# frankenz/Deep-convolutional-neural-network-ResNet-26-and-Attention-network

Measured on AMD Instinct MI355X. Metric: tiles/sec fwd+bwd, 256x256x3 bags, ResNet-26+attn, higher is better.
Workload: dtype bf16; 1 GPU; 8 bags x 256 tiles @256x256x3 per GPU, ResNet-26 (20/40/60/80) + attention-MIL head, fwd+bwd full-bag path (BASELINE.json configs[1]); global_bags=8, tiles_per_bag=256, tile=256, parallelism=bag-parallel dp1, one RCCL all-reduce of the flat 2.56 MB gradient bucket

## Files before the change

### deep-convolutional-neural-network-resnet-26-and-attention-network_amd/_lib.py

```python
import contextlib
import ctypes
import os
import subprocess
import threading

import torch

_HERE = os.path.dirname(os.path.abspath(__file__))
LIB_PATH = os.environ.get("MIL_LIB_PATH") or os.path.join(_HERE, "libmil_hip.so")
POISON_LIB_PATH = os.path.join(_HERE, "libmil_hip_poison.so")

MIL_DT_F32, MIL_DT_BF16, MIL_DT_BF16_DGRAD, MIL_DT_F32S, MIL_DT_F32S_DGRAD = 0, 1, 2, 3, 4
BF16X3 = "bf16x3"
PACK_FWD, PACK_DGRAD, PACK_STEM, PACK_DGRAD_S2 = 0, 1, 2, 3
_ERR = {1: "invalid argument", 2: "unsupported shape / channel configuration", 3: "kernel launch failed"}


class MilLibraryError(RuntimeError):
    pass


def build_library(verbose=False, poison=False):
    cmd = ["make", "-C", os.path.join(_HERE, "csrc"), "-j", str(min(8, os.cpu_count() or 1))] + (["POISON=1"] if poison else [])
    res = subprocess.run(cmd, stdout=subprocess.PIPE, stderr=subprocess.STDOUT, text=True)
    out = POISON_LIB_PATH if poison else os.path.join(_HERE, "libmil_hip.so")
    if verbose or res.returncode != 0:
        print(res.stdout)
    if res.returncode != 0:
        raise MilLibraryError(f"building {os.path.basename(out)} failed")
    return out


_c = ctypes
_vp, _i, _f, _sz = _c.c_void_p, _c.c_int, _c.c_float, _c.c_size_t
_SIGS = {
    "mil_abi_version": ([], _i),
    "mil_stream_copy": ([_vp, _vp, _sz, _vp], _i),
    "mil_split_probe": ([_vp, _vp, _vp, _i, _vp], _i),
    "mil_stem_s2d": ([_vp, _vp, _i, _i, _i, _i, _vp], _i),
    "mil_u8_decode_table": ([_vp], _i),
    "mil_stem_s2d_u8": ([_vp, _vp, _i, _i, _i, _i, _vp], _i),
    "mil_packed_weight_elems": ([_c.POINTER(_sz), _i, _i, _i, _i], _i),
    "mil_pack_conv_weights": ([_vp, _vp, _vp, _vp, _i, _i, _i, _i, _i, _vp], _i),
    "mil_conv_igemm": ([_vp] * 6 + [_i] * 12 + [_f, _i, _vp], _i),
    "mil_conv_wgrad_workspace": ([_c.POINTER(_sz)] + [_i] * 12, _i),
    "mil_conv_wgrad": ([_vp, _vp, _vp, _vp, _vp, _sz] + [_i] * 13 + [_vp], _i),
    "mil_reduce_job_bytes": ([], _i),
    "mil_reduce_defer_begin": ([_vp, _i], _i),
    "mil_reduce_defer_end": ([_c.POINTER(_i)], _i),
    "mil_wgrad_reduce_all": ([_vp, _vp, _i, _vp], _i),
    "mil_conv_bwd_fused_workspace": ([_c.POINTER(_sz)] + [_i] * 8, _i),
    "mil_conv_bwd_fused": ([_vp] * 8 + [_sz] + [_i] * 9 + [_f, _i, _vp], _i),
    "mil_maxpool_fwd": ([_vp, _vp, _vp, _i, _i, _i, _i, _i, _vp], _i),
    "mil_maxpool_bwd": ([_vp, _vp, _vp, _i, _i, _i, _i, _i, _f, _i, _vp], _i),
    "mil_resize_plan": ([_i, _i, _c.POINTER(_i)], _i),
    "mil_resize_coeffs": ([_i, _i, _vp, _vp], _i),
    "mil_tile_preprocess": ([_vp, _vp, _vp, _vp, _vp, _vp, _i, _i, _i, _i, _vp], _i),
    "mil_tile_preprocess_s2d": ([_vp, _vp, _vp, _vp, _vp, _vp, _i, _i, _i, _i, _vp], _i),
    "mil_tile_preprocess_u8": ([_vp, _vp, _vp, _vp, _vp, _vp, _i, _i, _i, _i, _vp], _i),
    "mil_tile_preprocess_win": ([_vp, _c.c_int64, _vp, _c.c_int64, _vp, _vp, _vp, _vp, _vp, _i, _i, _i, _i, _vp], _i),
    "mil_tile_preprocess_win_s2d": ([_vp, _c.c_int64, _vp, _c.c_int64, _vp, _vp, _vp, _vp, _vp, _i, _i, _i, _i, _vp], _i),
    "mil_tile_preprocess_win_u8": ([_vp, _c.c_int64, _vp, _c.c_int64, _vp, _vp, _vp, _vp, _vp, _i, _i, _i, _i, _vp], _i),
    "mil_roi_stats": ([_vp, _c.c_int64, _vp, _c.c_int64, _i, _i, _i, _i, _i, _vp, _vp], _i),
    "mil_stem_fwd_fused_xs": ([_vp, _vp, _vp, _vp, _vp, _i, _i, _i, _i, _f, _i, _vp], _i),
    "mil_stem_fwd_fused_u8": ([_vp, _vp, _vp, _vp, _vp, _i, _i, _i, _i, _f, _i, _vp], _i),
    "mil_conv_block_fwd": ([_vp, _vp, _vp, _vp, _vp, _vp, _vp, _i, _i, _i, _i, _f, _i, _vp], _i),
    "mil_conv_chain": ([_vp, _vp, _i, _i, _i, _i, _i, _f, _i, _vp], _i),
    "mil_conv_pair": ([_vp, _vp, _vp, _vp, _vp, _i, _vp, _vp, _vp, _vp, _vp, _i, _vp, _i, _i, _i, _i, _f, _i, _vp], _i),
    "mil_conv_s2_entry": ([_vp, _vp, _vp, _vp, _vp, _vp, _i, _i, _i, _i, _i, _f, _i, _vp], _i),
    "mil_conv_wgrad_pair_workspace": ([_c.POINTER(_sz), _i, _i, _i, _i, _i, _i, _i, _i], _i),
    "mil_conv_wgrad_pair": ([_vp, _vp, _vp, _vp, _vp, _vp, _vp, _sz, _i, _i, _i, _i, _i, _i, _i, _i, _i, _vp], _i),
    "mil_conv_dgrad_s2": ([_vp, _vp, _vp, _vp, _vp, _i, _i, _i, _i, _i, _i, _i, _f, _i, _vp], _i),
    "mil_stem_fwd_fused": ([_vp, _vp, _vp, _vp, _vp, _vp, _i, _i, _i, _i, _f, _i, _vp], _i),
    "mil_stem_bwd_fused_workspace": ([_c.POINTER(_sz), _i, _i, _i, _i], _i),
    "mil_stem_bwd_fused": ([_vp, _vp, _vp, _vp, _vp, _vp, _sz, _i, _i, _i, _f, _i, _i, _vp], _i),
    "mil_stem_bwd_fused_nchw_workspace": ([_c.POINTER(_sz), _i, _i, _i, _i], _i),
    "mil_stem_bwd_fused_nchw": ([_vp, _vp, _vp, _vp, _vp, _vp, _sz, _i, _i, _i, _f, _i, _i, _vp], _i),
    "mil_stem_bwd_fused_u8_workspace": ([_c.POINTER(_sz), _i, _i, _i, _i], _i),
    "mil_stem_bwd_fused_u8": ([_vp, _vp, _vp, _vp, _vp, _vp, _sz, _i, _i, _i, _f, _i, _i, _vp], _i),
# ... 99 lines not shown
```

### deep-convolutional-neural-network-resnet-26-and-attention-network_amd/csrc/conv_wgrad.hip

```cpp
#include "pf_common.cuh"
#include "reduce.cuh"
#include "stamp.cuh"
#include "u8_feed.cuh"

template <typename T>
struct WgradArgs {
    const typename T::elem* x;
    const typename T::elem* dz;
    float* slab;
    ConvGeom g;
    int ntiles;
    int tile_px;
    int lds_z_off;
    unsigned x_bytes, z_bytes;
    const typename T::elem* dz2;
    int lds_z2_off;
    unsigned long long* stamp;
};

__device__ __forceinline__ bf16x8_t tr_pair(const char* p0, const char* p1) {
    typedef __attribute__((address_space(3))) s16x4_t lds_s16x4;
    s16x4_t lo = __builtin_amdgcn_ds_read_tr16_b64_v4i16((lds_s16x4*)(p0));
    s16x4_t hi = __builtin_amdgcn_ds_read_tr16_b64_v4i16((lds_s16x4*)(p1));
    typedef __attribute__((ext_vector_type(8))) short s16x8_t;
    s16x8_t v = __builtin_shufflevector(lo, hi, 0, 1, 2, 3, 4, 5, 6, 7);
    return __builtin_bit_cast(bf16x8_t, v);
}

__host__ __device__ constexpr bool mil_wgrad_x3_half(bool split, int ks, int cinp, int nt, int msplit, bool proj) {
    return split && ks == 3 && cinp == 40 && nt == 3 && msplit == 1 && !proj;
}
__host__ __device__ constexpr int mil_wgrad_halo_max(int cinp, bool proj, bool split = false, bool half = false) {
    if ((split && cinp >= 64) || half) return 200;
    return (proj && cinp <= 24) ? 576 : 400;
}
__host__ __device__ constexpr int mil_wgrad_tile_max(int cinp, bool split, bool half = false) { return ((split && cinp >= 64) || half) ? 128 : 256; }
constexpr int MIL_WGRAD_X3_WAVES = 2;
template <typename T, int KS, int CINP, int NT, int MSPLIT, bool PF, int NW = 4, bool PROJ = false>
__global__ __launch_bounds__(64 * NW, NW == 8 ? ((T::SPLIT && CINP <= 24 && NT <= 2) ? MIL_WGRAD_X3_WAVES : 2) : ((PF && CINP > 40) ? 1 : ((PF && T::SPLIT) ? 2 : 0))) void wgrad_kernel(WgradArgs<T> a) {
    extern __shared__ __attribute__((aligned(16))) char smem[];
    MIL_POISON(smem);
    constexpr int ESZ = T::ESZ;
    constexpr int PIXB = mil_pix_pitch(CINP, ESZ);
    constexpr int COUTP = mil_nt_to_cp(NT);
    constexpr int PIXZ = mil_pix_pitch(COUTP, ESZ);
    constexpr int CG = CINP / 8;
    constexpr int RG = KS * KS * CG;
    constexpr int MT = (RG + 1) / 2;
    constexpr int MT_S = (MT + MSPLIT - 1) / MSPLIT;
    constexpr int NTHR = 64 * NW;
    constexpr int MW = (MT_S + NW - 1) / NW;
    constexpr int PM0 = 2 * CG, PM1 = (5 * CG - 1) / 2, PMN = PROJ ? PM1 - PM0 + 1 : 0;
    constexpr bool WPIPE = T::DT == MIL_DT_BF16 && PF && CINP < 64;
    constexpr bool ZFOLD = T::SPLIT && (COUTP % 16) == 8;
    constexpr int ZFOLD_D = COUTP * 2 - 16;
    const ConvGeom& g = a.g;
    const int tid = threadIdx.x, lane = tid & 63;
    const int wave = __builtin_amdgcn_readfirstlane(tid >> 6);
    const int split = blockIdx.y;
    const bool bias_wave = (wave == 0 && split == 0);
    char* ldsX = smem;
    char* ldsZ = smem + a.lds_z_off;

    int toff[MW];
    bool mvalid[MW];
    int proj_i = -1, proj_mt = 0;
#pragma unroll
    for (int i = 0; i < MW; ++i) {
        const int ml = wave + NW * i;
        const int mt = split * MT_S + ml;
        mvalid[i] = (ml < MT_S) && (mt < MT);
        if (PROJ && mvalid[i] && mt >= PM0 && mt <= PM1) { proj_i = i; proj_mt = mt; }
// ... 244 lines not shown
        if (ZFOLD && nt == NT - 1) {
            const float up = __shfl_down(v, 8, 16);
            return col < 8 ? v + up : 0.f;
        }
        return v;
    };
    if constexpr (PROJ) {
        if (proj_i >= 0) {
#pragma unroll
            for (int nt = 0; nt < NT; ++nt)
#pragma unroll
                for (int e = 0; e < 4; ++e)
                    slab[(size_t)((MT + 1 + proj_mt - PM0) * 16 + gq * 4 + e) * SLAB_COLS + nt * 16 + col] = unfold(accp[nt][e], nt);
        }
    }
#pragma unroll
    for (int i = 0; i < MW; ++i) {
        if (!mvalid[i]) continue;
        const int mt = split * MT_S + wave + NW * i;
#pragma unroll
        for (int nt = 0; nt < NT; ++nt)
#pragma unroll
            for (int e = 0; e < 4; ++e)
                slab[(size_t)(mt * 16 + gq * 4 + e) * SLAB_COLS + nt * 16 + col] = unfold(acc[i][nt][e], nt);
    }
    if (bias_wave) {
#pragma unroll
        for (int nt = 0; nt < NT; ++nt)
#pragma unroll
            for (int e = 0; e < 4; ++e)
                slab[(size_t)(MT * 16 + gq * 4 + e) * SLAB_COLS + nt * 16 + col] = unfold(accb[nt][e], nt);
    }
}

static thread_local MilDeferState g_defer{nullptr, 0, 0};
MilDeferState& mil_defer_state() { return g_defer; }

__global__ __launch_bounds__(32 * MIL_RED_GROUPS) void wgrad_reduce_job_kernel(MilReduceJob j) {
    __shared__ f32x4_t part[MIL_RED_GROUPS][32];
    MIL_POISON_STATIC(part);
    mil_reduce_job_block(j, blockIdx.x, part);
}

__global__ __launch_bounds__(32 * MIL_RED_GROUPS) void wgrad_reduce_all_kernel(const MilReduceJob* __restrict__ jobs, int njobs) {
    __shared__ f32x4_t part[MIL_RED_GROUPS][32];
    __shared__ int which;
    MIL_POISON_STATIC(part); MIL_POISON_STATIC(which);
    const int b = blockIdx.x;
    if (threadIdx.x < 64) {
        bool mine = false;
        if ((int)threadIdx.x < njobs) {
            const int b0 = jobs[threadIdx.x].block0, nb = jobs[threadIdx.x].n_blocks;
            mine = b >= b0 && b < b0 + nb;
        }
        const unsigned long long m = __ballot(mine);
        if (threadIdx.x == 0) which = m ? __ffsll((long long)m) - 1 : -1;
    }
    __syncthreads();
    const int k = which;
    if (k < 0) return;
    const MilReduceJob j = jobs[k];
    mil_reduce_job_block(j, b - j.block0, part);
}

extern "C" int mil_reduce_job_bytes(void) { return (int)sizeof(MilReduceJob); }

// ... 184 lines not shown
    if (g.ks == 4 && cinp == 16 && coutp == 24) MIL_WG(4, 16, 2, 1);
    if (g.ks == 4 && cinp == 16 && coutp == 64) MIL_WG(4, 16, 4, 1);
    if (g.ks == 3) {
        if (cinp == 24 && coutp == 24) MIL_WG(3, 24, 2, 1);
        if (cinp == 40 && coutp == 40) MIL_WG(3, 40, 3, 1);
        if (cinp == 64 && coutp == 64) MIL_WG(3, 64, 4, 1);
        if (cinp == 80 && coutp == 80) { if constexpr (T::SPLIT) { MIL_WG(3, 80, 5, 3); } else { MIL_WG(3, 80, 5, 2); } }
        if (cinp == 24 && coutp == 40) MIL_WG(3, 24, 3, 1);
        if (cinp == 40 && coutp == 64) {
            if constexpr (T::SPLIT) { MIL_WG(3, 40, 4, 2); } else { MIL_WG(3, 40, 4, 1); }
        }
        if (cinp == 64 && coutp == 80) MIL_WG(3, 64, 5, 2);
    }
    if (g.ks == 1) {
        if (cinp == 24 && coutp == 40) MIL_WG(1, 24, 3, 1);
        if (cinp == 40 && coutp == 64) MIL_WG(1, 40, 4, 1);
        if (cinp == 64 && coutp == 80) MIL_WG(1, 64, 5, 1);
    }
#undef MIL_WG
    return MIL_ERR_UNSUPPORTED;
}

static int wgrad_entry(const void* x, const void* dz, float* dw, float* db, void* ws, size_t ws_bytes, int n_img,
                       int H, int W, int cin, int Ho, int Wo, int cout, int ks, int stride, int pad, int stem_mode,
                       int accumulate, int dtype, bool query, size_t* need, void* stream) {
    if (n_img < 0 || H <= 0 || W <= 0 || Ho <= 0 || Wo <= 0) return MIL_ERR_ARG;
    ConvGeom g{};
    g.n_img = n_img; g.H = H; g.W = W; g.Ho = Ho; g.Wo = Wo; g.ks = ks; g.stride = stride; g.pad = pad; g.zins = 0;
    hipStream_t st = reinterpret_cast<hipStream_t>(stream);
    if (dtype == MIL_DT_BF16) return dispatch_wgrad<BF16>(x, dz, dw, db, ws, ws_bytes, g, cout, cin, stem_mode, accumulate, query, need, st);
    if (dtype == MIL_DT_F32) return dispatch_wgrad<F32>(x, dz, dw, db, ws, ws_bytes, g, cout, cin, stem_mode, accumulate, query, need, st);
    if (dtype == MIL_DT_F32S) return dispatch_wgrad<F32S>(x, dz, dw, db, ws, ws_bytes, g, cout, cin, stem_mode, accumulate, query, need, st);
    return MIL_ERR_ARG;
}

struct StemBwdArgs {
    const __bf16* xs;
    const float* x;
    const uint8_t* x8;
    int H, W;
    unsigned x_bytes;
    int lds_dump_off;
    const __bf16* gp;
    int gpx;
    const uint8_t* widx;
    float* slab;
    ConvGeom g;
    int Hp, Wp;
    int ntiles;
    int lds_z_off, lds_g_off, lds_i_off;
    unsigned xs_bytes, gp_bytes, wi_bytes;
    float slope;
    unsigned long long* stamp;
};

constexpr int MIL_STEM_BWD_WAVES = 2;
template <bool FROM_X, bool X3, int NPW, bool U8>
__device__ __forceinline__ void stem_bwd_fused_body(const StemBwdArgs& a) {
    extern __shared__ __attribute__((aligned(16))) char smem[];
    MIL_POISON(smem);
    static_assert(!X3 || FROM_X, "the split-precision form reads the fp32 tiles");
    static_assert(!U8 || FROM_X, "the uint8 feed rebuilds its s2d tiles");
    constexpr int CINP = 16, NT = 2, KS = 4, COUTP = 24;
    constexpr int PIXB = mil_pix_pitch(CINP, X3 ? 4 : 2);
    constexpr int PIXZ = mil_pix_pitch(COUTP, X3 ? 4 : 2);
    constexpr int PIXG = 96;
// ... 484 lines not shown
                                     reinterpret_cast<hipStream_t>(stream));
}

extern "C" int mil_conv_wgrad_pair_workspace(size_t* bytes, int n_img, int H, int W, int cin, int Ho, int Wo, int cout, int dtype) {
    if (!bytes) return MIL_ERR_ARG;
    return wgrad_pair_entry(nullptr, nullptr, nullptr, nullptr, nullptr, nullptr, nullptr, 0, n_img, H, W, cin, Ho, Wo, cout, 0,
                            dtype, true, bytes, nullptr);
}

extern "C" int mil_conv_wgrad_pair(const void* x, const void* dz1, const void* dz2, float* dw3, float* db3, float* dw1,
                                   void* workspace, size_t workspace_bytes, int n_img, int H, int W, int cin, int Ho, int Wo,
                                   int cout, int accumulate, int dtype, void* stream) {
    if (!x || !dz1 || !dz2 || !dw3 || !dw1 || !workspace) return MIL_ERR_ARG;
    size_t need = 0;
    return wgrad_pair_entry(x, dz1, dz2, dw3, db3, dw1, workspace, workspace_bytes, n_img, H, W, cin, Ho, Wo, cout, accumulate,
                            dtype, false, &need, stream);
}

extern "C" int mil_conv_wgrad_workspace(size_t* bytes, int n_img, int H, int W, int cin, int Ho, int Wo, int cout,
                                        int ks, int stride, int pad, int stem_mode, int dtype) {
    if (!bytes) return MIL_ERR_ARG;
    return wgrad_entry(nullptr, nullptr, nullptr, nullptr, nullptr, 0, n_img, H, W, cin, Ho, Wo, cout, ks, stride, pad,
                       stem_mode, 0, dtype, true, bytes, nullptr);
}

extern "C" int mil_conv_wgrad(const void* x, const void* dz, float* dw, float* db, void* workspace,
                              size_t workspace_bytes, int n_img, int H, int W, int cin, int Ho, int Wo, int cout,
                              int ks, int stride, int pad, int stem_mode, int accumulate, int dtype, void* stream) {
    if (!x || !dz || !dw) return MIL_ERR_ARG;
    size_t need = 0;
    return wgrad_entry(x, dz, dw, db, workspace, workspace_bytes, n_img, H, W, cin, Ho, Wo, cout, ks, stride, pad,
                       stem_mode, accumulate, dtype, false, &need, stream);
}
```

### deep-convolutional-neural-network-resnet-26-and-attention-network_amd/encoder.py

```python
import contextlib
import os

import torch
from torch import nn

from . import _lib as L
from . import hooks
from . import ops

STAGE_WIDTHS = (20, 40, 60, 80)
WEIGHT_EPOCH = [0]
STEM_WIDTH = 20


def invalidate_packed_weights():
    WEIGHT_EPOCH[0] += 1


class BasicResBlock(nn.Module):
    expansion = 1

    def __init__(self, inplanes, planes, stride=1, downsample=None, groups=1, base_width=64):
        super().__init__()
        if groups != 1 or base_width != 64:
# ... 5 lines not shown
        self.stride = stride

    def forward(self, x):
        raise RuntimeError("BasicResBlock is executed by the fused HIP encoder (ResNet.forward); "
                           "it has no stand-alone torch path")


class ResNet(nn.Module):

    def __init__(self, block=BasicResBlock, layers=(3, 3, 3, 3), num_classes=80, zero_init_residual=False,
                 groups=1, width_per_group=64, compute_dtype=L.BF16X3):
        super().__init__()
        if block is not BasicResBlock or groups != 1 or width_per_group != 64:
            raise ValueError("the HIP encoder implements BasicResBlock with groups=1, base_width=64")
        self.inplanes = STEM_WIDTH
        self.conv1 = nn.Conv2d(3, STEM_WIDTH, kernel_size=7, stride=2, padding=3)
        self.relu = nn.LeakyReLU(ops.LEAK, inplace=True)
        self.maxpool = nn.MaxPool2d(kernel_size=3, stride=2, padding=1)
        for i, (width, depth) in enumerate(zip(STAGE_WIDTHS, layers)):
            setattr(self, f"layer{i + 1}", self._make_layer(width, depth, stride=1 if i == 0 else 2))
        self.avgpool = nn.AdaptiveAvgPool2d((1, 1))
        self.fc = nn.Linear(STAGE_WIDTHS[-1], num_classes, bias=False)
        self.compute_dtype = compute_dtype
        self.overlap_wgrad = False
        self.direct_grad = False
        self.n_side_streams = 1
        self.fuse_backward = True
        self.fuse_stem_forward = True
        self.keep_s2d = False
        self.fuse_stage_entry = True
        self.fuse_block_forward = True
        self.dense_grads = True
        self.batch_reductions = True
        self._reduce_batch = None
        self._pack_table = None
        self._pack_version = None
        self._side = None

    def _make_layer(self, planes, blocks, stride=1):
        shortcut = None
        if stride != 1 or self.inplanes != planes:
            shortcut = nn.Sequential(nn.Conv2d(self.inplanes, planes, kernel_size=1, stride=stride, bias=False))
        seq = [BasicResBlock(self.inplanes, planes, stride, shortcut)]
        self.inplanes = planes
        seq += [BasicResBlock(planes, planes) for _ in range(1, blocks)]
        return nn.Sequential(*seq)

    def blocks(self):
        for i in range(4):
            for blk in getattr(self, f"layer{i + 1}"):
                yield blk

    def encoder_params(self):
        ps = [self.conv1.weight, self.conv1.bias]
        for blk in self.blocks():
            ps += [blk.conv1.weight, blk.conv1.bias, blk.conv2.weight, blk.conv2.bias]
            if blk.downsample is not None:
                ps.append(blk.downsample[0].weight)
        ps.append(self.fc.weight)
        return ps

    def _side_streams(self):
        if self._side is None:
            self._side = [torch.cuda.Stream() for _ in range(self.n_side_streams)]
        return self._side

# ... 261 lines not shown
    batch = None
    if net.batch_reductions and not use_side:
        if net._reduce_batch is None or net._reduce_batch.device != dfeats.device:
            net._reduce_batch = ops.ReduceBatch(dfeats.device)
        batch = net._reduce_batch

    def gout(*params):
        return tuple(None if p is None else p.grad for p in params) if direct else None

    def wgrad(xin, dzz, cin, cout, key=None, **kw):
        n, h, w, _ = xin.shape
        _, ho, wo, _ = dzz.shape
        need = ops.wgrad_workspace_bytes(n, h, w, cin, ho, wo, cout, kw["ks"], kw["stride"], kw["pad"],
                                         kw.get("stem", False), xin.dtype)
        if batch is not None:
            assert key is not None, "deferred reductions need one workspace per call site: pass key="
            return ops.conv_wgrad(xin, dzz, cin, cout, workspace=batch.workspace(("w", key), need), **kw)
        if not use_side:
            if ws[-1] is None or ws[-1].numel() * 4 < need:
                ws[-1] = torch.empty((need + 3) // 4, dtype=torch.float32, device=xin.device)
            return ops.conv_wgrad(xin, dzz, cin, cout, workspace=ws[-1], **kw)
        k = rr[0] % len(sides)
        rr[0] += 1
        side = sides[k]
        side.wait_stream(main)
        with torch.cuda.stream(side):
            if ws[k] is None or ws[k].numel() * 4 < need:
                ws[k] = torch.empty((need + 3) // 4, dtype=torch.float32, device=xin.device)
            out = ops.conv_wgrad(xin, dzz, cin, cout, workspace=ws[k], **kw)
        xin.record_stream(side)
        dzz.record_stream(side)
        return out

    fws = None

    def is_dense(t, c):
        return t.shape[-1] == c and ops.cpad(c) != c

    def fused_bwd(dzz, wd, xin, cin, cout, addend, mask, out, key=None):
        nonlocal fws
        n, h, w, _ = dzz.shape
        dense = is_dense(dzz, cout)
        need = ops.bwd_fused_workspace_bytes(n, h, w, cout, cin, 3, 1, dzz.dtype, dense)
        if need is None:
            if dense:
                raise RuntimeError("dense gradient layout chosen for a shape without a fused backward kernel")
            return None
        if batch is not None:
            return ops.conv_bwd_fused(dzz, wd, xin, cin, cout, addend=addend, mask=mask, workspace=batch.workspace(("f", key), need), out=out)
        if fws is None or fws.numel() * 4 < need:
            fws = torch.empty((need + 3) // 4, dtype=torch.float32, device=dzz.device)
        return ops.conv_bwd_fused(dzz, wd, xin, cin, cout, addend=addend, mask=mask, workspace=fws, out=out)

    def stage_dgrad_chain(bi, dz_out):
        li, j, depth = net.block_position(bi)
        e = bi - depth + 1
        split_ = dtype == torch.float32 and L.dt_code(dtype, mma=True) == L.MIL_DT_F32S
        if j != depth - 1 or depth < 2 or depth > 3 or not net.fuse_backward or not (dtype == torch.bfloat16 or split_):
            return None
        ent = blocks[e]
        if ent.stride != 2 or ent.downsample is None or any(b.stride != 1 or b.downsample is not None for b in blocks[e + 1:bi + 1]):
            return None
        cout = ent.conv1.out_channels
        n, h, w, cp = dz_out.shape
        if (cp, h, w) not in ops.RESIDENT_SHAPES or ops.bwd_fused_workspace_bytes(n, h, w, cout, cout, 3, 1, dtype) is not None:
            return None
        convs, src = [], None
        for k in range(bi, e, -1):
            xin_k, o1_k, _ = saved["blocks"][k]
            w2d_k, _ = net._packed(f"b{k}.c2", blocks[k].conv2.weight, None, L.PACK_DGRAD, dtype)
            w1d_k, _ = net._packed(f"b{k}.c1", blocks[k].conv1.weight, None, L.PACK_DGRAD, dtype)
            convs.append(dict(w=w2d_k, act=o1_k))
            convs.append(dict(w=w1d_k, res=dz_out if src is None else src, act=xin_k))
            src = len(convs) - 1
        _xin_e, o1_e, _ = saved["blocks"][e]
        w2d_e, _ = net._packed(f"b{e}.c2", ent.conv2.weight, None, L.PACK_DGRAD, dtype)
        convs.append(dict(w=w2d_e, act=o1_e))
        outs = ops.conv_chain(dz_out, convs)
        if outs is None:
            return None
        done = {}
        dz_k = dz_out
        for i, k in enumerate(range(bi, e, -1)):
            xin_k, o1_k, _ = saved["blocks"][k]
            dmid_k, dz_prev = outs[2 * i], outs[2 * i + 1]
            grads[f"b{k}.c2"] = wgrad(o1_k, dz_k, cout, cout, key=(k, 2), ks=3, stride=1, pad=1, out=gout(blocks[k].conv2.weight, blocks[k].conv2.bias))
            grads[f"b{k}.c1"] = wgrad(xin_k, dmid_k, cout, cout, key=(k, 1), ks=3, stride=1, pad=1, out=gout(blocks[k].conv1.weight, blocks[k].conv1.bias))
            done[k] = "done"
            dz_k = dz_prev
        grads[f"b{e}.c2"] = wgrad(o1_e, dz_k, cout, cout, key=(e, 2), ks=3, stride=1, pad=1, out=gout(ent.conv2.weight, ent.conv2.bias))
        done[e] = (dz_k, outs[-1])
        return done

    pre = {}
    with (batch if batch is not None else contextlib.nullcontext()):
        for bi in range(len(blocks) - 1, -1, -1):
            blk = blocks[bi]
            xin, o1, _out = saved["blocks"][bi]
            cin, cout, s = blk.conv1.in_channels, blk.conv1.out_channels, blk.stride
            if bi not in pre:
                chain = stage_dgrad_chain(bi, dz)
                if chain is not None:
                    pre.update(chain)
            if pre.get(bi) == "done":
                continue
            w2d, _ = net._packed(f"b{bi}.c2", blk.conv2.weight, None, L.PACK_DGRAD, dtype)
            if bi in pre:
                dz, dz1 = pre[bi]
                fused = "chain"
            else:
                fused = fused_bwd(dz, w2d, o1, cout, cout, None, True, gout(blk.conv2.weight, blk.conv2.bias), key=(bi, 2)) if net.fuse_backward else None
            if fused == "chain":
                pass
            elif fused is not None:
                dz1, grads[f"b{bi}.c2"] = fused[0], (fused[1], fused[2])
            elif is_dense(dz, cout):
                raise RuntimeError("dense gradient layout without the fused backward")
            else:
                grads[f"b{bi}.c2"] = wgrad(o1, dz, cout, cout, key=(bi, 2), ks=3, stride=1, pad=1, out=gout(blk.conv2.weight, blk.conv2.bias))
                if s == 1 and blk.downsample is None and net.fuse_backward:
                    w1d_, _ = net._packed(f"b{bi}.c1", blk.conv1.weight, None, L.PACK_DGRAD, dtype)
                    chain = ops.conv_pair(dz, w2d, None, w1d_, None, actA=o1, resB=dz, actB=xin if bi > 0 else None)
                    if chain is not None:
# ... 106 lines not shown
```

### deep-convolutional-neural-network-resnet-26-and-attention-network_amd/ops.py

```python
import ctypes

import torch

from . import _lib as L

LEAK = 0.1


class KernelTimer:

    def __init__(self, want):
        self.want = want
        self.spans = []

    def bracket(self, label):
        if not self.want(label):
            return None
        start = torch.cuda.Event(enable_timing=True)
        end = torch.cuda.Event(enable_timing=True)
        start.record()
        self.spans.append((label, start, end))
        return end

    def durations_ms(self):
# ... 129 lines not shown


def wgrad_workspace_bytes(n, h, w, cin, ho, wo, cout, ks, stride, pad, stem, dtype):
    need = ctypes.c_size_t(0)
    L.check(L.lib().mil_conv_wgrad_workspace(ctypes.byref(need), n, h, w, cin, ho, wo, cout, ks, stride, pad,
                                             1 if stem else 0, L.dt_code(dtype, mma=True)), "mil_conv_wgrad_workspace")
    return need.value


def conv_wgrad(x, dz, cin, cout, *, ks, stride, pad, stem=False, want_bias=True, workspace=None, out=None):
    n, h, w, cin_p = x.shape
    _, ho, wo, cout_p = dz.shape
    _need(dz, (n, ho, wo, cpad(cout)), x.dtype, "dz")
    _need(x, (n, h, w, 16 if stem else cpad(cin)), x.dtype, "x")
    need = wgrad_workspace_bytes(n, h, w, cin, ho, wo, cout, ks, stride, pad, stem, x.dtype)
    if workspace is None or workspace.numel() * workspace.element_size() < need:
        workspace = torch.empty((need + 3) // 4, dtype=torch.float32, device=x.device)
    kk = 7 if stem else ks
    if out is None:
        dw = torch.empty((cout, cin, kk, kk), dtype=torch.float32, device=x.device)
        db = torch.empty(cout, dtype=torch.float32, device=x.device) if want_bias else None
    else:
        dw, db = out
        _need(dw, (cout, cin, kk, kk), torch.float32, "dw")
        _need(db, (cout,), torch.float32, "db")
    end = TIMER.bracket(("wgrad", cin_p, cout_p, ks, stride, n, ho, wo)) if TIMER else None
    L.check(L.lib().mil_conv_wgrad(x.data_ptr(), dz.data_ptr(), dw.data_ptr(), L.ptr(db), workspace.data_ptr(),
                                   workspace.numel() * workspace.element_size(), n, h, w, cin, ho, wo, cout, ks, stride,
                                   pad, 1 if stem else 0, 0 if out is None else 1, L.dt_code(x.dtype, mma=True), L.stream_ptr()),
            "mil_conv_wgrad")
    if end is not None:
        end.record()
    return dw, db


def bwd_fused_workspace_bytes(n, h, w, cout, cin, ks, pad, dtype, dense=False):
    need = ctypes.c_size_t(0)
    rc = L.lib().mil_conv_bwd_fused_workspace(ctypes.byref(need), n, h, w, cout, cin, ks, pad, L.dt_code(dtype, dense, mma=True))
    if rc == 2:
        return None
    L.check(rc, "mil_conv_bwd_fused_workspace")
    return need.value


def conv_bwd_fused(dz, wpack_dgrad, x, cin, cout, *, addend=None, mask=True, ks=3, pad=1, workspace=None, slope=LEAK,
                   out=None):
    n, h, w, cz = dz.shape
    dense = cz == cout and cpad(cout) != cout
    need = bwd_fused_workspace_bytes(n, h, w, cout, cin, ks, pad, dz.dtype, dense)
    if need is None:
        return None
    _need(dz, (n, h, w, cout if dense else cpad(cout)), dz.dtype, "dz")
    _need(x, (n, h, w, cpad(cin)), dz.dtype, "x")
    _need(addend, (n, h, w, cin if dense else cpad(cin)), dz.dtype, "addend")
    if workspace is None or workspace.numel() * workspace.element_size() < need:
        workspace = torch.empty((need + 3) // 4, dtype=torch.float32, device=dz.device)
    dx = torch.empty((n, h, w, cin), dtype=dz.dtype, device=dz.device) if dense else torch.empty_like(x)
    if out is None:
        dw = torch.empty((cout, cin, ks, ks), dtype=torch.float32, device=dz.device)
        db = torch.empty(cout, dtype=torch.float32, device=dz.device)
    else:
        dw, db = out
        _need(dw, (cout, cin, ks, ks), torch.float32, "dw")
        _need(db, (cout,), torch.float32, "db")
    end = TIMER.bracket(("bwd_fused", cpad(cout), cpad(cin), ks, 1, False, n, h, w, addend is not None)) if TIMER else None
    L.check(L.lib().mil_conv_bwd_fused(dz.data_ptr(), wpack_dgrad.data_ptr(), x.data_ptr(), L.ptr(addend), dx.data_ptr(),
# ... 486 lines not shown
```

### include/mil_hip.h

```cpp
#ifndef MIL_HIP_H
#define MIL_HIP_H

#include <stddef.h>
#include <stdint.h>

#ifdef __cplusplus
extern "C" {
#endif

#define MIL_OK 0
#define MIL_ERR_ARG 1
#define MIL_ERR_UNSUPPORTED 2
#define MIL_ERR_LAUNCH 3

#define MIL_DT_F32 0
#define MIL_DT_BF16 1
#define MIL_DT_BF16_DGRAD 2
#define MIL_DT_F32S 3
#define MIL_DT_F32S_DGRAD 4

#define MIL_PACK_FWD 0
#define MIL_PACK_DGRAD 1
#define MIL_PACK_STEM 2
#define MIL_PACK_DGRAD_S2 3

int mil_abi_version(void);

int mil_stream_copy(void* dst, const void* src, size_t bytes, void* stream);
int mil_split_probe(const float* v, uint16_t* hi, uint16_t* lo, int n, void* stream);

int mil_stem_s2d(const float* x_nchw, void* out, int n, int H, int W, int dtype, void* stream);

int mil_u8_decode_table(float* out256);
int mil_stem_s2d_u8(const uint8_t* x_u8, void* out, int n, int H, int W, int dtype, void* stream);

int mil_packed_weight_elems(size_t* elems, int cout, int cin, int ks, int mode);
int mil_pack_conv_weights(const float* w, const float* bias, void* wpack, float* bias_pad, int cout, int cin,
                          int ks, int mode, int dtype, void* stream);

int mil_conv_igemm(const void* x, const void* wpack, const float* bias_pad, const void* res, const void* act,
                   void* y, int n_img, int H, int W, int cin_p, int Ho, int Wo, int cout_p, int ks, int stride,
                   int pad, int zero_insert, int apply_lrelu, float slope, int dtype, void* stream);

int mil_conv_wgrad_workspace(size_t* bytes, int n_img, int H, int W, int cin, int Ho, int Wo, int cout, int ks,
                             int stride, int pad, int stem_mode, int dtype);
int mil_conv_wgrad(const void* x, const void* dz, float* dw, float* db, void* workspace, size_t workspace_bytes,
                   int n_img, int H, int W, int cin, int Ho, int Wo, int cout, int ks, int stride, int pad,
                   int stem_mode, int accumulate, int dtype, void* stream);

int mil_reduce_job_bytes(void);
int mil_reduce_defer_begin(void* jobs_host, int max_jobs);
int mil_reduce_defer_end(int* njobs);
int mil_wgrad_reduce_all(const void* jobs_dev, const void* jobs_host, int njobs, void* stream);

int mil_conv_bwd_fused_workspace(size_t* bytes, int n_img, int H, int W, int cout, int cin, int ks, int pad, int dtype);
int mil_conv_bwd_fused(const void* dz, const void* wpack_dgrad, const void* x, const void* addend, void* dx, float* dw,
                       float* db, void* workspace, size_t workspace_bytes, int n_img, int H, int W, int cout, int cin,
                       int ks, int pad, int apply_mask, int accumulate, float slope, int dtype, void* stream);

int mil_maxpool_fwd(const void* x, void* y, uint8_t* widx, int n, int H, int W, int cp, int dtype, void* stream);
int mil_maxpool_bwd(const void* gy, const uint8_t* widx, void* gx, int n, int H, int W, int cp,
                    int apply_lrelu_mask, float slope, int dtype, void* stream);

int mil_resize_plan(int in_size, int out_size, int* ksize);
int mil_resize_coeffs(int in_size, int out_size, int32_t* bounds, int32_t* kk);
int mil_tile_preprocess(const uint8_t* rois, const int32_t* params, const int32_t* bounds_host, const int32_t* bounds_dev,
                        const int32_t* kk_dev, float* out, int T, int S, int pad, int R, void* stream);
int mil_tile_preprocess_s2d(const uint8_t* rois, const int32_t* params, const int32_t* bounds_host, const int32_t* bounds_dev,
                            const int32_t* kk_dev, void* xs, int T, int S, int pad, int R, void* stream);
int mil_tile_preprocess_u8(const uint8_t* rois, const int32_t* params, const int32_t* bounds_host, const int32_t* bounds_dev,
                           const int32_t* kk_dev, uint8_t* out, int T, int S, int pad, int R, void* stream);
int mil_tile_preprocess_win(const uint8_t* base, int64_t base_bytes, const int64_t* win_off_dev, int64_t row_pitch,
                            const int32_t* params, const int32_t* bounds_host, const int32_t* bounds_dev,
                            const int32_t* kk_dev, float* out, int T, int S, int pad, int R, void* stream);
int mil_tile_preprocess_win_s2d(const uint8_t* base, int64_t base_bytes, const int64_t* win_off_dev, int64_t row_pitch,
                                const int32_t* params, const int32_t* bounds_host, const int32_t* bounds_dev,
                                const int32_t* kk_dev, void* xs, int T, int S, int pad, int R, void* stream);
int mil_tile_preprocess_win_u8(const uint8_t* base, int64_t base_bytes, const int64_t* win_off_dev, int64_t row_pitch,
                               const int32_t* params, const int32_t* bounds_host, const int32_t* bounds_dev,
                               const int32_t* kk_dev, uint8_t* out, int T, int S, int pad, int R, void* stream);

// ... 103 lines not shown
```

Measured before the change: 257,600 tiles/s.

## Batch same-shape stage wgrad convolutions into one multi-job kernel launch

```diff
diff --git a/deep-convolutional-neural-network-resnet-26-and-attention-network_amd/_lib.py b/deep-convolutional-neural-network-resnet-26-and-attention-network_amd/_lib.py
--- a/deep-convolutional-neural-network-resnet-26-and-attention-network_amd/_lib.py
+++ b/deep-convolutional-neural-network-resnet-26-and-attention-network_amd/_lib.py
@@ -45,6 +45,8 @@
     "mil_conv_igemm": ([_vp] * 6 + [_i] * 12 + [_f, _i, _vp], _i),
     "mil_conv_wgrad_workspace": ([_c.POINTER(_sz)] + [_i] * 12, _i),
     "mil_conv_wgrad": ([_vp, _vp, _vp, _vp, _vp, _sz] + [_i] * 13 + [_vp], _i),
+    "mil_conv_wgrad_batch_workspace": ([_c.POINTER(_sz)] + [_i] * 9, _i),
+    "mil_conv_wgrad_batch": ([_vp, _i, _i, _vp], _i),
     "mil_reduce_job_bytes": ([], _i),
     "mil_reduce_defer_begin": ([_vp, _i], _i),
     "mil_reduce_defer_end": ([_c.POINTER(_i)], _i),
diff --git a/deep-convolutional-neural-network-resnet-26-and-attention-network_amd/csrc/conv_wgrad.hip b/deep-convolutional-neural-network-resnet-26-and-attention-network_amd/csrc/conv_wgrad.hip
--- a/deep-convolutional-neural-network-resnet-26-and-attention-network_amd/csrc/conv_wgrad.hip
+++ b/deep-convolutional-neural-network-resnet-26-and-attention-network_amd/csrc/conv_wgrad.hip
@@ -2,6 +2,8 @@
 #include "reduce.cuh"
 #include "stamp.cuh"
 #include "u8_feed.cuh"
+
+#define MIL_WGRAD_BATCH_MAX 8
 
 template <typename T>
 struct WgradArgs {
@@ -36,8 +38,9 @@
 }
 __host__ __device__ constexpr int mil_wgrad_tile_max(int cinp, bool split, bool half = false) { return ((split && cinp >= 64) || half) ? 128 : 256; }
 constexpr int MIL_WGRAD_X3_WAVES = 2;
+#define MIL_WGRAD_BOUNDS __launch_bounds__(64 * NW, NW == 8 ? ((T::SPLIT && CINP <= 24 && NT <= 2) ? MIL_WGRAD_X3_WAVES : 2) : ((PF && CINP > 40) ? 1 : ((PF && T::SPLIT) ? 2 : 0)))
 template <typename T, int KS, int CINP, int NT, int MSPLIT, bool PF, int NW = 4, bool PROJ = false>
-__global__ __launch_bounds__(64 * NW, NW == 8 ? ((T::SPLIT && CINP <= 24 && NT <= 2) ? MIL_WGRAD_X3_WAVES : 2) : ((PF && CINP > 40) ? 1 : ((PF && T::SPLIT) ? 2 : 0))) void wgrad_kernel(WgradArgs<T> a) {
+__device__ __forceinline__ void wgrad_body(const WgradArgs<T>& a) {
     extern __shared__ __attribute__((aligned(16))) char smem[];
     MIL_POISON(smem);
     constexpr int ESZ = T::ESZ;
@@ -348,6 +351,30 @@
                 slab[(size_t)(MT * 16 + gq * 4 + e) * SLAB_COLS + nt * 16 + col] = unfold(accb[nt][e], nt);
     }
 }
+
+template <typename T, int KS, int CINP, int NT, int MSPLIT, bool PF, int NW = 4, bool PROJ = false>
+__global__ MIL_WGRAD_BOUNDS void wgrad_kernel(WgradArgs<T> a) {
+    wgrad_body<T, KS, CINP, NT, MSPLIT, PF, NW, PROJ>(a);
+}
+
+template <typename T>
+struct WgradBatchArgs {
+    WgradArgs<T> a;
+    const typename T::elem* x[MIL_WGRAD_BATCH_MAX];
+    const typename T::elem* dz[MIL_WGRAD_BATCH_MAX];
+    float* slab[MIL_WGRAD_BATCH_MAX];
+};
+
+template <typename T, int KS, int CINP, int NT, int MSPLIT, bool PF, int NW = 4>
+__global__ MIL_WGRAD_BOUNDS void wgrad_batch_kernel(WgradBatchArgs<T> b) {
+    WgradArgs<T> a = b.a;
+    const int job = blockIdx.z;
+#pragma unroll
+    for (int k = 1; k < MIL_WGRAD_BATCH_MAX; ++k)
+        if (job == k) { a.x = b.x[k]; a.dz = b.dz[k]; a.slab = b.slab[k]; }
+    wgrad_body<T, KS, CINP, NT, MSPLIT, PF, NW, false>(a);
+}
+#undef MIL_WGRAD_BOUNDS
 
 static thread_local MilDeferState g_defer{nullptr, 0, 0};
 MilDeferState& mil_defer_state() { return g_defer; }
@@ -598,6 +625,89 @@
     if (dtype == MIL_DT_F32) return dispatch_wgrad<F32>(x, dz, dw, db, ws, ws_bytes, g, cout, cin, stem_mode, accumulate, query, need, st);
     if (dtype == MIL_DT_F32S) return dispatch_wgrad<F32S>(x, dz, dw, db, ws, ws_bytes, g, cout, cin, stem_mode, accumulate, query, need, st);
     return MIL_ERR_ARG;
+}
+
+struct MilWgradJob {
+    const void* x; const void* dz; float* dw; float* db; void* workspace; size_t workspace_bytes;
+    int n_img, H, W, cin, Ho, Wo, cout, accumulate;
+};
+
+template <typename T, int KS, int CINP, int NT, int MSPLIT>
+static int run_wgrad_batch(const MilWgradJob* jobs, int njobs, ConvGeom g, int cout, int cin, bool query, size_t* need,
+                           hipStream_t stream) {
+    constexpr bool PF_OK = T::TR16 && (!T::SPLIT || CINP < 64 || (CINP == 64 || (CINP == 80 && MSPLIT >= 3)));
+    if constexpr (!PF_OK) return MIL_ERR_UNSUPPORTED;
+    else {
+    WgradPlan pl{};
+    int lds_z_off = 0;
+    int rc = plan_wgrad<T, KS, CINP, NT, MSPLIT>(g, pl, &lds_z_off, false);
+    if (rc != MIL_OK) return rc;
+    constexpr bool HALF = mil_wgrad_x3_half(T::SPLIT, KS, CINP, NT, MSPLIT, false);
+    constexpr int NW = HALF ? 4 : ((CINP >= 64 || T::SPLIT) ? 8 : 4);
+    const size_t xb_total = (size_t)g.n_img * g.H * g.W * CINP * T::ESZ;
+    const size_t zb_total = (size_t)g.n_img * g.Ho * g.Wo * mil_nt_to_cp(NT) * T::ESZ;
+    const bool pf = (((g.hh * g.hw) << g.ti_log2) <= mil_wgrad_halo_max(CINP, false, T::SPLIT, HALF)) &&
+                    (1 << pl.tile_px_log2) <= mil_wgrad_tile_max(CINP, T::SPLIT, HALF) && g.hh < 1024 && g.hw < 1024;
+    if (!pf || g.n_img < 1 || xb_total > mil_buffer_limit() || zb_total > mil_buffer_limit()) return MIL_ERR_UNSUPPORTED;
+    auto kern1 = wgrad_kernel<T, KS, CINP, NT, MSPLIT, true, NW, false>;
+    auto kern = wgrad_batch_kernel<T, KS, CINP, NT, MSPLIT, true, NW>;
+    const int nthr = 64 * NW;
+    g.n_groups = (g.n_img + (1 << g.ti_log2) - 1) >> g.ti_log2;
+    const int ntiles = g.n_groups * g.tiles_y * g.tiles_x;
+    int gx = mil_num_cus() * mil_resident_per_cu(kern1, pl.lds, 2, nthr) / (MSPLIT * njobs);
+    if (gx > ntiles) gx = ntiles;
+    if (gx < 1) gx = 1;
+    const size_t bytes = pl.slab_elems * gx * sizeof(float);
+    if (query) { *need = bytes; return MIL_OK; }
+    for (int k = 0; k < njobs; ++k)
+        if (jobs[k].workspace_bytes < bytes) return MIL_ERR_ARG;
+    if (pl.lds > 64 * 1024) {
+        if (hipFuncSetAttribute(reinterpret_cast<const void*>(kern), hipFuncAttributeMaxDynamicSharedMemorySize, pl.lds) != hipSuccess)
+            return MIL_ERR_LAUNCH;
+    }
+    WgradBatchArgs<T> b{};
+    b.a.g = g; b.a.ntiles = ntiles; b.a.tile_px = 1 << pl.tile_px_log2; b.a.lds_z_off = lds_z_off;
+    b.a.lds_z2_off = lds_z_off + (1 << pl.tile_px_log2) * mil_pix_pitch(mil_nt_to_cp(NT), T::ESZ);
+    b.a.x_bytes = (unsigned)xb_total; b.a.z_bytes = (unsigned)zb_total;
+    for (int k = 0; k < MIL_WGRAD_BATCH_MAX; ++k) {
+        const MilWgradJob& j = jobs[k < njobs ? k : 0];
+        b.x[k] = (const typename T::elem*)j.x; b.dz[k] = (const typename T::elem*)j.dz; b.slab[k] = (float*)j.workspace;
+    }
+    b.a.x = b.x[0]; b.a.dz = b.dz[0]; b.a.slab = b.slab[0];
+    hipLaunchKernelGGL(kern, dim3(gx, MSPLIT, njobs), dim3(nthr), pl.lds, stream, b);
+    MIL_CHECK_LAUNCH();
+    for (int k = 0; k < njobs; ++k) {
+        MilReduceJob j{};
+        j.slab = (const float*)jobs[k].workspace; j.nslab = gx; j.slab_elems = pl.slab_elems; j.slab_cols = pl.slab_cols;
+        j.n_rows = KS * KS * CINP; j.dw = jobs[k].dw; j.db = jobs[k].db; j.cout = cout; j.cin = cin; j.ks = KS; j.kind = 0;
+        j.cinp = CINP; j.stem_mode = 0; j.bias_row = pl.mt * 16; j.accumulate = jobs[k].accumulate;
+        mil_reduce_or_defer(j, stream);
+        MIL_CHECK_LAUNCH();
+    }
+    return MIL_OK;
+    }
+}
+
+static int wgrad_batch_entry(const MilWgradJob* jobs, int njobs, const MilWgradJob& g0, int dtype, bool query, size_t* need,
+                             void* stream) {
+    if (njobs < 1 || g0.n_img < 0 || g0.H <= 0 || g0.W <= 0 || g0.Ho <= 0 || g0.Wo <= 0 || g0.cin <= 0 || g0.cout <= 0) return MIL_ERR_ARG;
+    if (njobs > MIL_WGRAD_BATCH_MAX) return MIL_ERR_UNSUPPORTED;
+    for (int k = 0; !query && k < njobs; ++k) {
+        const MilWgradJob& j = jobs[k];
+        if (!j.x || !j.dz || !j.dw || !j.workspace) return MIL_ERR_ARG;
+        if (j.n_img != g0.n_img || j.H != g0.H || j.W != g0.W || j.cin != g0.cin || j.Ho != g0.Ho || j.Wo != g0.Wo || j.cout != g0.cout)
+            return MIL_ERR_UNSUPPORTED;
+    }
+    if (g0.Ho != g0.H || g0.Wo != g0.W) return MIL_ERR_UNSUPPORTED;
+    ConvGeom g{};
+    g.n_img = g0.n_img; g.H = g0.H; g.W = g0.W; g.Ho = g0.Ho; g.Wo = g0.Wo; g.ks = 3; g.stride = 1; g.pad = 1; g.zins = 0;
+    hipStream_t st = reinterpret_cast<hipStream_t>(stream);
+    const int cinp = mil_cpad(g0.cin), coutp = mil_cpad(g0.cout);
+    if (cinp == 80 && coutp == 80) {
+        if (dtype == MIL_DT_BF16) return run_wgrad_batch<BF16, 3, 80, 5, 2>(jobs, njobs, g, g0.cout, g0.cin, query, need, st);
+        if (dtype == MIL_DT_F32S) return run_wgrad_batch<F32S, 3, 80, 5, 3>(jobs, njobs, g, g0.cout, g0.cin, query, need, st);
+    }
+    return MIL_ERR_UNSUPPORTED;
 }
 
 struct StemBwdArgs {
@@ -1148,3 +1258,17 @@
     return wgrad_entry(x, dz, dw, db, workspace, workspace_bytes, n_img, H, W, cin, Ho, Wo, cout, ks, stride, pad,
                        stem_mode, accumulate, dtype, false, &need, stream);
 }
+
+extern "C" int mil_conv_wgrad_batch_workspace(size_t* bytes, int njobs, int n_img, int H, int W, int cin, int Ho, int Wo,
+                                              int cout, int dtype) {
+    if (!bytes) return MIL_ERR_ARG;
+    MilWgradJob g0{};
+    g0.n_img = n_img; g0.H = H; g0.W = W; g0.cin = cin; g0.Ho = Ho; g0.Wo = Wo; g0.cout = cout;
+    return wgrad_batch_entry(nullptr, njobs, g0, dtype, true, bytes, nullptr);
+}
+
+extern "C" int mil_conv_wgrad_batch(const MilWgradJob* jobs, int njobs, int dtype, void* stream) {
+    if (!jobs || njobs < 1) return MIL_ERR_ARG;
+    size_t need = 0;
+    return wgrad_batch_entry(jobs, njobs, jobs[0], dtype, false, &need, stream);
+}
diff --git a/deep-convolutional-neural-network-resnet-26-and-attention-network_amd/encoder.py b/deep-convolutional-neural-network-resnet-26-and-attention-network_amd/encoder.py
--- a/deep-convolutional-neural-network-resnet-26-and-attention-network_amd/encoder.py
+++ b/deep-convolutional-neural-network-resnet-26-and-attention-network_amd/encoder.py
@@ -61,6 +61,7 @@
         self.fuse_block_forward = True
         self.dense_grads = True
         self.batch_reductions = True
+        self.batch_wgrad = True
         self._reduce_batch = None
         self._pack_table = None
         self._pack_version = None
@@ -388,6 +389,31 @@
         dzz.record_stream(side)
         return out
 
+    def wgrad_batch(jobs, c):
+        def run(alloc):
+            return ops.conv_wgrad_batch([dict(x=xj, dz=dj, cin=c, cout=c, out=gout(cv.weight, cv.bias)) for _n, xj, dj, _k, cv in jobs],
+                                        ws_alloc=alloc)
+        if batch is not None:
+            return run(lambda k, nb: batch.workspace(("wb", jobs[k][3]), nb))
+
+        def alloc(k, nb, slot):
+            per = (nb + 3) // 4
+            if ws[slot] is None or ws[slot].numel() < per * len(jobs):
+                ws[slot] = torch.empty(per * len(jobs), dtype=torch.float32, device=jobs[0][1].device)
+            return ws[slot][k * per:(k + 1) * per]
+        if not use_side:
+            return run(lambda k, nb: alloc(k, nb, -1))
+        slot = rr[0] % len(sides)
+        rr[0] += 1
+        side = sides[slot]
+        side.wait_stream(main)
+        with torch.cuda.stream(side):
+            out = run(lambda k, nb: alloc(k, nb, slot))
+        for _n, xj, dj, _k, _cv in jobs:
+            xj.record_stream(side)
+            dj.record_stream(side)
+        return out
+
     fws = None
 
     def is_dense(t, c):
@@ -437,14 +463,19 @@
             return None
         done = {}
         dz_k = dz_out
+        jobs = []
         for i, k in enumerate(range(bi, e, -1)):
             xin_k, o1_k, _ = saved["blocks"][k]
             dmid_k, dz_prev = outs[2 * i], outs[2 * i + 1]
-            grads[f"b{k}.c2"] = wgrad(o1_k, dz_k, cout, cout, key=(k, 2), ks=3, stride=1, pad=1, out=gout(blocks[k].conv2.weight, blocks[k].conv2.bias))
-            grads[f"b{k}.c1"] = wgrad(xin_k, dmid_k, cout, cout, key=(k, 1), ks=3, stride=1, pad=1, out=gout(blocks[k].conv1.weight, blocks[k].conv1.bias))
+            jobs.append((f"b{k}.c2", o1_k, dz_k, (k, 2), blocks[k].conv2))
+            jobs.append((f"b{k}.c1", xin_k, dmid_k, (k, 1), blocks[k].conv1))
             done[k] = "done"
             dz_k = dz_prev
-        grads[f"b{e}.c2"] = wgrad(o1_e, dz_k, cout, cout, key=(e, 2), ks=3, stride=1, pad=1, out=gout(ent.conv2.weight, ent.conv2.bias))
+        jobs.append((f"b{e}.c2", o1_e, dz_k, (e, 2), ent.conv2))
+        batched = wgrad_batch(jobs, cout) if net.batch_wgrad else None
+        for i, (name, xin_j, dz_j, key, conv) in enumerate(jobs):
+            grads[name] = batched[i] if batched is not None else \
+                wgrad(xin_j, dz_j, cout, cout, key=key, ks=3, stride=1, pad=1, out=gout(conv.weight, conv.bias))
         done[e] = (dz_k, outs[-1])
         return done
 
diff --git a/deep-convolutional-neural-network-resnet-26-and-attention-network_amd/ops.py b/deep-convolutional-neural-network-resnet-26-and-attention-network_amd/ops.py
--- a/deep-convolutional-neural-network-resnet-26-and-attention-network_amd/ops.py
+++ b/deep-convolutional-neural-network-resnet-26-and-attention-network_amd/ops.py
@@ -185,6 +185,61 @@
     if end is not None:
         end.record()
     return dw, db
+
+
+class _WgradJob(ctypes.Structure):
+    _fields_ = [("x", ctypes.c_void_p), ("dz", ctypes.c_void_p), ("dw", ctypes.c_void_p), ("db", ctypes.c_void_p),
+                ("workspace", ctypes.c_void_p), ("workspace_bytes", ctypes.c_size_t)] + \
+               [(f, ctypes.c_int) for f in ("n_img", "H", "W", "cin", "Ho", "Wo", "cout", "accumulate")]
+
+
+WGRAD_BATCH_MAX = 8
+
+
+def conv_wgrad_batch(jobs, *, want_bias=True, ws_alloc=None):
+    if not 1 <= len(jobs) <= WGRAD_BATCH_MAX:
+        return None
+    x0, dz0 = jobs[0]["x"], jobs[0]["dz"]
+    code = L.dt_code(x0.dtype, mma=True)
+    n, h, w, _ = x0.shape
+    need = ctypes.c_size_t(0)
+    rc = L.lib().mil_conv_wgrad_batch_workspace(ctypes.byref(need), len(jobs), n, h, w, jobs[0]["cin"], dz0.shape[1], dz0.shape[2],
+                                                jobs[0]["cout"], code)
+    if rc == 2:
+        return None
+    L.check(rc, "mil_conv_wgrad_batch_workspace")
+    arr = (_WgradJob * len(jobs))()
+    outs, keep = [], []
+    for k, j in enumerate(jobs):
+        x, dz, cin, cout = j["x"], j["dz"], j["cin"], j["cout"]
+        if x.dim() != 4 or dz.dim() != 4 or x.dtype != x0.dtype or x.device != x0.device:
+            return None
+        nk, hk, wk, _ = x.shape
+        _need(x, (nk, hk, wk, cpad(cin)), x0.dtype, "x")
+        _need(dz, (nk, dz.shape[1], dz.shape[2], cpad(cout)), x0.dtype, "dz")
+        if j.get("out") is None:
+            dw = torch.empty((cout, cin, 3, 3), dtype=torch.float32, device=x.device)
+            db = torch.empty(cout, dtype=torch.float32, device=x.device) if want_bias else None
+        else:
+            dw, db = j["out"]
+            _need(dw, (cout, cin, 3, 3), torch.float32, "dw")
+            _need(db, (cout,), torch.float32, "db")
+        ws = ws_alloc(k, need.value) if ws_alloc is not None else torch.empty((need.value + 3) // 4, dtype=torch.float32, device=x.device)
+        keep.append(ws)
+        a = arr[k]
+        a.x, a.dz, a.dw, a.db, a.workspace = x.data_ptr(), dz.data_ptr(), dw.data_ptr(), L.ptr(db), ws.data_ptr()
+        a.workspace_bytes = ws.numel() * ws.element_size()
+        a.n_img, a.H, a.W, a.cin, a.Ho, a.Wo, a.cout = nk, hk, wk, cin, dz.shape[1], dz.shape[2], cout
+        a.accumulate = 0 if j.get("out") is None else 1
+        outs.append((dw, db))
+    end = TIMER.bracket(("wgrad_batch", x0.shape[3], dz0.shape[3], len(jobs), n, h, w)) if TIMER else None
+    rc = L.lib().mil_conv_wgrad_batch(ctypes.addressof(arr), len(jobs), code, L.stream_ptr())
+    if rc == 2:
+        return None
+    L.check(rc, "mil_conv_wgrad_batch")
+    if end is not None:
+        end.record()
+    return outs
 
 
 def bwd_fused_workspace_bytes(n, h, w, cout, cin, ks, pad, dtype, dense=False):
diff --git a/include/mil_hip.h b/include/mil_hip.h
--- a/include/mil_hip.h
+++ b/include/mil_hip.h
@@ -47,6 +47,21 @@
 int mil_conv_wgrad(const void* x, const void* dz, float* dw, float* db, void* workspace, size_t workspace_bytes,
                    int n_img, int H, int W, int cin, int Ho, int Wo, int cout, int ks, int stride, int pad,
                    int stem_mode, int accumulate, int dtype, void* stream);
+
+#define MIL_WGRAD_BATCH_MAX 8
+typedef struct MilWgradJob {
+    const void* x;
+    const void* dz;
+    float* dw;
+    float* db;
+    void* workspace;
+    size_t workspace_bytes;
+    int n_img, H, W, cin, Ho, Wo, cout;
+    int accumulate;
+} MilWgradJob;
+int mil_conv_wgrad_batch_workspace(size_t* bytes, int njobs, int n_img, int H, int W, int cin, int Ho, int Wo, int cout,
+                                   int dtype);
+int mil_conv_wgrad_batch(const MilWgradJob* jobs, int njobs, int dtype, void* stream);
 
 int mil_reduce_job_bytes(void);
 int mil_reduce_defer_begin(void* jobs_host, int max_jobs);
```

New measurement: 260,100 tiles/s (median of 6 runs). About the same (+1.0%).
